# NVlabs/nvdiffrecmc

Measured on NVIDIA H100. Metric: shadow_rays_per_second_train_step, higher is better.
Workload: dtype f32

## Files before the change

### nvdiffrecmc_b200/csrc/envshade.cu

```cuda
#include "bsdf.cuh"
#include "bvh_traverse.cuh"
#include "ctx.h"
#include "exact.cuh"
#include <vector>

namespace {

constexpr float MIN_ROUGHNESS = 0.08f;

struct ShadeParams {
    TView pos, nrm, view, kd, ks, diff_grad, spec_grad;
    const float *light; int l_s1, l_s2, l_s3; int Hl, Wl;
    uint32_t *rec_count;
    float *rec_rays;
    int rec_slots;
    int B, H, W;
    uint32_t bsdf; float shadow_scale, sample_frac;
    float *pos_grad, *nrm_grad, *kd_grad, *ks_grad, *light_grad;
};

struct EnvParams : ShadeParams {
    TView mask, ro;
    const float *pdf; int p_s1, p_s2;
    const float *rows; int r_s;
// ... 103 lines not shown
__device__ __forceinline__ xf3 x_toworld(xf3 a, const PixelFrame &f) { return f.U * a.x + f.V * a.y + f.W * a.z; }

__device__ __forceinline__ float ggx_pdf_value(const PixelFrame &f, f3 wi)
{
    const f3 wo_l = toF3(f.wo_l_raw);
    const xf3 wi_lx = x_tolocal(X3(wi), f);
    const f3 wi_l = toF3(wi_lx);
    float pdf = 0.0f;
    if (wo_l.z > 0.0f && wi_l.z > 0.0f) {
        const f3 m = toF3(xnormalize(wi_lx + f.wo_l_raw));
        float woDotH = dot(m, wo_l);
        float alpha = f.alpha.v;
        float D = eval_ndf_ggx(alpha, m.z);
        float G1 = eval_g1_ggx(alpha * alpha, wo_l.z);
        pdf = G1 * D * fmaxf(0.0f, woDotH) / wo_l.z;
        pdf /= (4.0f * woDotH);
    }
    return pdf;
}
__device__ __forceinline__ void update_pdf(float &pdf, float opdf, float b) { if (b > 0.000001f) pdf += opdf * b; }

__device__ __forceinline__ float bsdf_pdf_value(const PixelFrame &f, xf3 wi)
{
    xf NdotL = xdot(f.N, wi);
    if (xmin(f.NdotV, NdotL).v < 1e-6f) return 1.0f;
    float pdf = 0.0f;
    float pD = f.pDiffuse.v;
    if (pD > 0.0f) update_pdf(pdf, fmaxf(NdotL.v, 0.0f) * MCS_INV_PI, pD);
    if (f.pSpecular.v > 0.0f) update_pdf(pdf, ggx_pdf_value(f, toF3(wi)), 1.0f - pD);
    return pdf;
}

__device__ __forceinline__ xf3 bsdf_sample(const PixelFrame &f, xf sx, xf sy, xf sz, float &pdf)
{
    pdf = 0.0f;
    const float pD = f.pDiffuse.v;
    xf3 wi;
    if (sz < f.pDiffuse) {
        if (pD < 0.0001f) { pdf = 1.0f; return f.N; }
        xf phi = xf(__double2float_rn(xd_mul(2.0 * XD_PI, (double)sx.v)));
        xf ct = xsqrt(sy);
        xf st = xf(__double2float_rn(__dsqrt_rn(__dsub_rn(1.0, (double)sy.v))));
        xf sp, cp;
        det_sincos(phi, sp, cp);
        xf3 vec = f.U * (cp * st) + f.V * (sp * st) + f.W * ct;
        wi = xnormalize(vec);
        pdf = fmaxf(0.000001f, ct.v * MCS_INV_PI) * pD;
        if (f.pSpecular.v > 0.0f) update_pdf(pdf, ggx_pdf_value(f, toF3(wi)), 1.0f - pD);
    } else {
        if (!(f.wo_l.z.v > 0.0f)) { pdf = 0.0f; wi = X3(xf(0.0f), xf(0.0f), xf(0.0f)); }
        else {
            const xf alpha = f.alpha;
            xf3 Vh = xnormalize(X3(alpha * f.wo_l.x, alpha * f.wo_l.y, f.wo_l.z));
            xf3 T1 = (Vh.z.v < 0.9999f) ? xnormalize(xcross(X3(xf(0.0f), xf(0.0f), xf(1.0f)), Vh)) : X3(xf(1.0f), xf(0.0f), xf(0.0f));
            xf3 T2 = xcross(Vh, T1);
            xf r = xsqrt(sx);
            xf phi = (xf(2.0f) * xf(MCS_PI)) * sy;
            xf sp, cp;
            det_sincos(phi, sp, cp);
            xf t1 = r * cp, t2 = r * sp;
            xf s = xf(0.5f) * (xf(1.0f) + Vh.z);
            t2 = (xf(1.0f) - s) * xsqrt(xf(1.0f) - t1 * t1) + s * t2;
            xf3 Nh = T1 * t1 + T2 * t2 + Vh * xsqrt(xmax(xf(0.0f), xf(1.0f) - t1 * t1 - t2 * t2));
            xf3 h = xnormalize(X3(alpha * Nh.x, alpha * Nh.y, xmax(xf(0.0f), Nh.z)));
            xf woDotH = xdot(f.wo_l, h);
            xf3 wi_l = h * woDotH * xf(2.0f) - f.wo_l;
            wi = xnormalize(x_toworld(wi_l, f));
            float a = alpha.v, woz = f.wo_l.z.v;
            float G1 = eval_g1_ggx(a * a, woz);
            float D = eval_ndf_ggx(a, h.z.v);
            pdf = G1 * D * fmaxf(0.0f, woDotH.v) / woz;
            pdf /= (4.0f * woDotH.v);
        }
        pdf *= 1.0f - pD;
        if (pD > 0.0f) update_pdf(pdf, fmaxf(xdot(f.N, wi).v, 0.0f) * MCS_INV_PI, pD);
    }
    return wi;
}

__device__ __forceinline__ float warp_sum(float v)
{
#pragma unroll
    for (int o = 16; o > 0; o >>= 1) v += __shfl_xor_sync(0xFFFFFFFFu, v, o);
    return v;
}

struct ShadeAcc { f3 D, S, kd, ks, nrm, wo; };

template <bool BWD>
__device__ __forceinline__ void shade_ray(const ShadeParams &p, const f3 nrm, const f3 kd, const f3 ks, const f3 wo, const f3 dgrad, const f3 sgrad,
                                          const f3 wi, const float mis, const uint32_t tex, ShadeAcc &a)
{
    const bool diffuse_only = (p.bsdf == 1u || p.bsdf == 2u);
    const int tx = tex & 0xFFFFu, ty = (tex >> 16) & 0x7FFFu;
    const float wgt = ((tex >> 31) ? 1.0f - p.shadow_scale : 1.0f) * mis * p.sample_frac;
    const float *lp = p.light + (size_t)ty * p.l_s1 + (size_t)tx * p.l_s2;
    const f3 light_col = F3(__ldg(lp), __ldg(lp + p.l_s3), __ldg(lp + 2 * p.l_s3));
    float diffv = 0.0f; f3 specv = F3(0.0f);
    if (!BWD) {
        if (diffuse_only) diffv = fwd_lambert(nrm, wi);
        else ox_fwd_pbr_bsdf(kd, ks, wo, nrm, wi, MIN_ROUGHNESS, diffv, specv);
        a.D += light_col * (diffv * wgt);
        a.S += specv * light_col * wgt;
        return;
    }
    const f3 dD = dgrad * light_col * wgt, dS = sgrad * light_col * wgt;
    ox_fwdbwd_pbr_bsdf(diffuse_only, kd, ks, wo, nrm, wi, MIN_ROUGHNESS, sum(dD), dS, diffv, specv, a.kd, a.ks, a.wo, a.nrm);
    const f3 lg = F3(__fmaf_rn(dgrad.x, diffv, __fmul_rn(sgrad.x, specv.x)), __fmaf_rn(dgrad.y, diffv, __fmul_rn(sgrad.y, specv.y)),
                     __fmaf_rn(dgrad.z, diffv, __fmul_rn(sgrad.z, specv.z))) * wgt;
    float *gp = p.light_grad + ((size_t)ty * p.Wl + tx) * 3;
    if (lg.x != 0.0f) atomicAdd(gp, lg.x);
    if (lg.y != 0.0f) atomicAdd(gp + 1, lg.y);
    if (lg.z != 0.0f) atomicAdd(gp + 2, lg.z);
}

__device__ __forceinline__ void store_pixel_grads(const ShadeParams &p, const int64_t pix, const f3 pos, const f3 view, const ShadeAcc &a, const int lane)
{
    const float v[12] = {a.kd.x, a.kd.y, a.kd.z, a.ks.x, a.ks.y, a.ks.z, a.nrm.x, a.nrm.y, a.nrm.z, a.wo.x, a.wo.y, a.wo.z};
    const bool b4 = (lane >> 4) & 1, b3 = (lane >> 3) & 1;
    float h[6], t[3];
#pragma unroll
    for (int i = 0; i < 6; ++i) h[i] = (b4 ? v[6 + i] : v[i]) + __shfl_xor_sync(0xFFFFFFFFu, b4 ? v[i] : v[6 + i], 16);
#pragma unroll
    for (int i = 0; i < 3; ++i) t[i] = (b3 ? h[3 + i] : h[i]) + __shfl_xor_sync(0xFFFFFFFFu, b3 ? h[i] : h[3 + i], 8);
#pragma unroll
    for (int o = 4; o > 0; o >>= 1) {
#pragma unroll
        for (int i = 0; i < 3; ++i) t[i] += __shfl_xor_sync(0xFFFFFFFFu, t[i], o);
    }
    if ((lane & 7) == 0) {
        const int which = lane >> 3;
        float *g = (which == 0 ? p.kd_grad : which == 1 ? p.ks_grad : which == 2 ? p.nrm_grad : p.pos_grad) + pix * 3;
        if (which == 3) {
            f3 d__wo = F3(0.0f);
            bwd_safe_normalize(view - pos, d__wo, F3(t[0], t[1], t[2]));
            t[0] = -d__wo.x; t[1] = -d__wo.y; t[2] = -d__wo.z;
        }
        g[0] = t[0]; g[1] = t[1]; g[2] = t[2];
    }
}

__device__ __forceinline__ void zero_pixel_grads(const ShadeParams &p, const int64_t pix)
{
    float *a = p.pos_grad + pix * 3, *b = p.nrm_grad + pix * 3, *c = p.kd_grad + pix * 3, *d = p.ks_grad + pix * 3;
    a[0] = a[1] = a[2] = 0.0f; b[0] = b[1] = b[2] = 0.0f; c[0] = c[1] = c[2] = 0.0f; d[0] = d[1] = d[2] = 0.0f;
}

#ifndef MCS_REPLAY_MINB
#define MCS_REPLAY_MINB 32
#endif
#ifndef MCS_CTA_WARPS
#define MCS_CTA_WARPS 8
#endif
#ifndef MCS_STREAM_RECORD
#define MCS_STREAM_RECORD 1
#endif
#ifndef MCS_SPLIT_WALKS
#define MCS_SPLIT_WALKS 1
#endif
#ifndef MCS_SPLIT_BELOW
#define MCS_SPLIT_BELOW 20
#endif
#ifndef MCS_QSTACK
#define MCS_QSTACK 100
#endif
#ifndef MCS_LEAF_BATCH
#define MCS_LEAF_BATCH 32
#endif
#ifndef MCS_REFILL_BELOW
#define MCS_REFILL_BELOW 24
#endif
#ifndef MCS_COUNT_TRAVERSAL
#define MCS_COUNT_TRAVERSAL 0
#endif
#if MCS_COUNT_TRAVERSAL
__device__ unsigned long long g_trace_counts[3];
#endif
constexpr int NW = MCS_CTA_WARPS;
constexpr int SEG = 128;
constexpr int QTOT = NW * SEG;
#ifndef MCS_PCAP
#define MCS_PCAP 160
#endif
constexpr int PCAP = MCS_PCAP;
constexpr int PIXRING = 256;
static_assert(QTOT <= 65536, "queue entry index is stored in 16 bits");
static_assert(SEG <= 256 && SEG % 32 == 0, "sample slot within a fill is stored in 8 bits");

struct BlockQueue {
    float dx[QTOT], dy[QTOT], dz[QTOT], mis[QTOT];
    uint32_t tex[QTOT];
    uint16_t vlist[QTOT];
    uint8_t qitem[QTOT];
    uint32_t hitw[NW][SEG / 32];
    uint2 pl[NW][PCAP];
    float ro[NW][3];
    float rog[NW][3];
    float wo[NW][3];
    int pixid[NW];
    int seg_cnt[NW];
    int seg_head[NW];
    int pixring[PIXRING];
    int ring_head, ring_tail, more_chunks;
};
struct BlockQueueRec { uint32_t slot[QTOT]; };

struct PixelIn {
    f3 ro, pos, nrm, view, kd, ks;
    int ix, iy, iz;
    int64_t pix;
};

__device__ __forceinline__ PixelIn load_pixel(const EnvParams &p, int64_t pix)
{
    PixelIn q;
    q.pix = pix;
    q.ix = (int)(pix % p.W);
    const int64_t tt = pix / p.W;
    q.iy = (int)(tt % p.H); q.iz = (int)(tt / p.H);
    q.ro = p.ro.ld3(q.iz, q.iy, q.ix);
    q.pos = p.pos.ld3(q.iz, q.iy, q.ix);
    q.nrm = p.nrm.ld3(q.iz, q.iy, q.ix);
    q.view = p.view.ld3(q.iz, q.iy, q.ix);
    q.kd = p.kd.ld3(q.iz, q.iy, q.ix);
    q.ks = p.ks.ld3(q.iz, q.iy, q.ix);
    return q;
}

__device__ __forceinline__ void make_frame(const PixelIn &q, PixelFrame &f)
{
    f.N = X3(q.nrm);
    f.alpha = xf(q.ks.y) * xf(q.ks.y);
    f.wo = xnormalize(X3(q.view) - X3(q.pos));
    xf metallic = xf(q.ks.z);
    xf3 base = X3(q.kd);
    xf om = xf(1.0f) - metallic;
    xf3 specColor = X3(xf(0.04f) * om + base.x * metallic, xf(0.04f) * om + base.y * metallic, xf(0.04f) * om + base.z * metallic);
    xf lum = base.x * xf(0.2126f) + base.y * xf(0.7152f) + base.z * xf(0.0722f);
    xf diffuseWeight = om * lum;
    f.W = xnormalize(f.N);
    xONB(f.W, f.U, f.V);
    f.wo_l_raw = x_tolocal(f.wo, f);
    f.wo_l = xnormalize(f.wo_l_raw);
    xf specularWeight = xf(0.0f);
    if (f.wo_l.z.v > 0.0f) {
        xf c = xclamp(f.wo_l.z, xf(1e-4f), xf(1.0f) - xf(1e-4f));
        xf o = xf(1.0f) - c;
        xf o2 = o * o;
        xf scale = (o2 * o2) * o;
        xf os = xf(1.0f) - scale;
        xf3 F = X3(specColor.x * os + scale, specColor.y * os + scale, specColor.z * os + scale);
        specularWeight = F.x * xf(0.2126f) + F.y * xf(0.7152f) + F.z * xf(0.0722f);
    }
    xf sumw = diffuseWeight + specularWeight;
    f.pDiffuse = sumw.v > 0.0f ? diffuseWeight / sumw : xf(1.0f);
    f.pSpecular = xf(1.0f) - f.pDiffuse;
    f.NdotV = xdot(f.N, f.wo);
}

struct RayQ {
    float ax, ay, az, bx, by, bz;
    uint32_t nx, ny, nz, fx, fy, fz;
};
__device__ __forceinline__ float rcp_approx(float x) { float r; asm("rcp.approx.ftz.f32 %0, %1;" : "=f"(r) : "f"(x)); return r; }
__device__ __forceinline__ RayQ rayq_fetch(const float *__restrict__ g, const float *rog, float dx, float dy, float dz)
{
    RayQ r;
    const float ix = rcp_approx(fabsf(dx) < 1e-20f ? copysignf(1e-20f, dx) : dx);
    const float iy = rcp_approx(fabsf(dy) < 1e-20f ? copysignf(1e-20f, dy) : dy);
    const float iz = rcp_approx(fabsf(dz) < 1e-20f ? copysignf(1e-20f, dz) : dz);
    r.ax = __ldg(g + 3) * ix; r.ay = __ldg(g + 4) * iy; r.az = __ldg(g + 5) * iz;
    r.bx = fmaf(-8388608.0f, r.ax, rog[0] * ix);
    r.by = fmaf(-8388608.0f, r.ay, rog[1] * iy);
    r.bz = fmaf(-8388608.0f, r.az, rog[2] * iz);
    r.nx = dx < 0.0f ? 0x7432u : 0x7410u; r.ny = dy < 0.0f ? 0x7432u : 0x7410u; r.nz = dz < 0.0f ? 0x7432u : 0x7410u;
    r.fx = dx < 0.0f ? 0x7410u : 0x7432u; r.fy = dy < 0.0f ? 0x7410u : 0x7432u; r.fz = dz < 0.0f ? 0x7410u : 0x7432u;
    return r;
}
__device__ __forceinline__ float qplane(uint32_t w, uint32_t sel)
{
    uint32_t r;
    asm("prmt.b32 %0, %1, %2, %3;" : "=r"(r) : "r"(w), "r"(0x4B000000u), "r"(sel));
    return __uint_as_float(r);
}
__device__ __forceinline__ bool qslab(const uint4 c, const RayQ &r)
{
    const float a0 = fmaf(qplane(c.x, r.nx), r.ax, r.bx), a1 = fmaf(qplane(c.x, r.fx), r.ax, r.bx);
    const float b0 = fmaf(qplane(c.y, r.ny), r.ay, r.by), b1 = fmaf(qplane(c.y, r.fy), r.ay, r.by);
    const float c0 = fmaf(qplane(c.z, r.nz), r.az, r.bz), c1 = fmaf(qplane(c.z, r.fz), r.az, r.bz);
    const float tn = fmaxf(fmaxf(a0, b0), fmaxf(c0, 0.0f));
    const float tf = fminf(fminf(a1, b1), c1);
    return tn <= tf;
}

template <int MODE>
__device__ __forceinline__ void gen_segment(const EnvParams &p, BlockQueue &q, BlockQueueRec *qr, const PixelIn &px, const PixelFrame &f,
                                            int seg, int w0, int w1, int &qn, const int lane)
{
    const int S = p.S;
    const int qb = seg * SEG;
    const xf strata_frac = xf(1.0f) / xf((float)(unsigned)p.N);
    uint32_t s_seed = p.seed + (p.seed_dev ? __ldg(p.seed_dev) : 0u), s_pix = (uint32_t)(((px.iz + p.batch_offset) * p.H + px.iy) * p.W + px.ix);
    uint32_t rng = rand_pcg(s_seed) ^ rand_pcg(s_pix);
    const uint32_t lightIdx = rand_pcg(rng) % p.n_perms;
    const uint32_t bsdfIdx = rand_pcg(rng) % p.n_perms;
    const uint32_t rng2 = rng;
    const f3 nrm = px.nrm;

    for (int base = w0; base < w1; base += 32) {
        const int w = base + lane;
        const bool valid = w < w1;
        const bool is_bsdf = w >= S;
        const int i = is_bsdf ? w - S : w;
        xf3 dir = X3(xf(0.0f), xf(0.0f), xf(1.0f));
        float pdf_sum = 1.0f, pdf_b = 0.0f;
        int tx = 0, ty = 0;
        if (valid) {
            const uint2 sk = __ldg(p.skip + 5 * i + (is_bsdf ? 2 : 0));
            uint32_t st = rng2 * sk.x + sk.y;
            const uint32_t row = is_bsdf ? bsdfIdx : lightIdx;
            const uint32_t perm = (uint32_t)__ldg(p.perms + (size_t)row * p.pm_s1 + (size_t)i * p.pm_s3);
            const xf sx = (xf((float)(perm % (uint32_t)p.N)) + uniform_pcg(st)) * strata_frac;
            const xf sy = (xf((float)(perm / (uint32_t)p.N)) + uniform_pcg(st)) * strata_frac;
            if (!is_bsdf) {
                uint32_t cyi, cxi;
                xf ry = sample_cdf(p.rows, p.r_s, p.Hl, p.m_rows, sy, cyi);
                xf rx = sample_cdf(p.cols + (size_t)cyi * p.c_s1, p.c_s2, p.Wl, p.m_cols, sx, cxi);
                dir = tc_to_dir((xf((float)cxi) + rx) / xf((float)p.Wl), (xf((float)cyi) + ry) / xf((float)p.Hl));
            } else {
                const xf sz = uniform_pcg(st);
                dir = bsdf_sample(f, sx, sy, sz, pdf_b);
            }
            if (MODE == 2) {
                float cy;
                dir_to_texel(p, dir, tx, ty, cy);
                pdf_sum = light_pdf_value(p, tx, ty, cy) + (is_bsdf ? pdf_b : bsdf_pdf_value(f, dir));
            }
        }
        const f3 wi = toF3(dir);
        const bool live = valid && dot(nrm, wi) > 0.0f;
        if (MODE == 2 && valid) {
            const size_t rec = (size_t)px.pix * (2 * S) + (size_t)(2 * i + (is_bsdf ? 1 : 0));
            p.rec_texel[rec] = (ty << 16) | tx;
            if (!live) p.rec_vis[rec] = 2;
        }
        const unsigned m = __ballot_sync(0xFFFFFFFFu, live);
        if (live) {
            const int e = qb + qn + __popc(m & ((1u << lane) - 1u));
            q.dx[e] = wi.x; q.dy[e] = wi.y; q.dz[e] = wi.z;
            if (MODE == 2) {
                q.mis[e] = 1.0f / fmaxf(pdf_sum, 0.0001f);
                q.tex[e] = (uint32_t)((ty << 16) | tx);
                qr->slot[e] = (uint32_t)(2 * i + (is_bsdf ? 1 : 0));
            } else {
                q.mis[e] = pdf_b;
                q.tex[e] = is_bsdf ? 1u : 0u;
            }
            q.qitem[e] = (uint8_t)(w - w0);
        }
        qn += __popc(m);
    }
    if (MODE != 2) {
        __syncwarp();
        for (int e0 = 0; e0 < qn; e0 += 32) {
            const int e = qb + e0 + lane;
            if (e0 + lane < qn) {
                const xf3 dir = X3(xf(q.dx[e]), xf(q.dy[e]), xf(q.dz[e]));
                int tx, ty; float cy;
                dir_to_texel(p, dir, tx, ty, cy);
                const float pdf_sum = light_pdf_value(p, tx, ty, cy) + (q.tex[e] ? q.mis[e] : bsdf_pdf_value(f, dir));
                q.mis[e] = 1.0f / fmaxf(pdf_sum, 0.0001f);
                q.tex[e] = (uint32_t)((ty << 16) | tx);
            }
        }
    }
}

__device__ __forceinline__ void trace_queue(const EnvParams &p, BlockQueue &q, const int warp, const int lane)
{
    constexpr int REFILL_BELOW = MCS_REFILL_BELOW;
    constexpr int LEAF_BATCH = MCS_LEAF_BATCH;
    unsigned lt;
    asm("mov.u32 %0, %%lanemask_lt;" : "=r"(lt));
    int pend = 0;
    int my = -1;
    int node = 0, sp = 0, sb = 0;
    int stack[MCS_QSTACK];
    RayQ r; r.ax = r.ay = r.az = 1.0f; r.bx = r.by = r.bz = 0.0f; r.nx = r.ny = r.nz = 0x7410u; r.fx = r.fy = r.fz = 0x7432u;
    const BvhView b = p.bvh;
    uint2 *pl = q.pl[warp];
    int seg = warp, exhausted = 0;
#if MCS_COUNT_TRAVERSAL
    unsigned long long n_rays = 0, n_visits = 0, n_tests = 0;
#endif

    auto leaf_batch = [&](int n) {
        __syncwarp();
        const int base = pend - n;
        if (lane < n) {
            const uint2 ent = pl[base + lane];
            const int e = (int)ent.x;
            if (!(q.tex[e] >> 31)) {
                const int code = (int)ent.y;
                const int start = code >> 3, cnt = (code & 7) + 1;
                const int ps = e / SEG;
                const f3 o = F3(q.ro[ps][0], q.ro[ps][1], q.ro[ps][2]);
                const f3 d = F3(q.dx[e], q.dy[e], q.dz[e]);
                bool hit = false;
                for (int k = 0; k < cnt && !hit; ++k) {
#if MCS_COUNT_TRAVERSAL
                    ++n_tests;
#endif
                    const float4 *t = b.tris + 3 * (size_t)(start + k);
                    const float4 t0 = __ldg(t), t1 = __ldg(t + 1), t2 = __ldg(t + 2);
                    float tt, uu, vv;
                    hit = mt_hit(o, d, F3(t0.x, t0.y, t0.z), F3(t1.x, t1.y, t1.z), F3(t2.x, t2.y, t2.z), MCS_TMAX, tt, uu, vv);
                }
                if (hit) atomicOr(&q.tex[e], 0x80000000u);
            }
        }
        pend = base;
        __syncwarp();
    };

    while (true) {
        unsigned idle = __ballot_sync(0xFFFFFFFFu, my < 0);
        while (idle && exhausted < NW) {
            const int need = __popc(idle);
            int base = 0;
            if (lane == 0) base = atomicAdd(&q.seg_head[seg], need);
            base = __shfl_sync(0xFFFFFFFFu, base, 0);
            const int avail = q.seg_cnt[seg] - base;
            if (avail <= 0) { seg = seg + 1 == NW ? 0 : seg + 1; ++exhausted; continue; }
            const int take = avail < need ? avail : need;
            const int rank = __popc(idle & lt);
            if (my < 0 && rank < take) {
                const int idx = seg * SEG + base + rank;
                my = idx;
                r = rayq_fetch(b.qgrid, q.rog[seg], q.dx[idx], q.dy[idx], q.dz[idx]);
                node = 0; sp = 0; sb = 0;
#if MCS_COUNT_TRAVERSAL
                ++n_rays;
#endif
            }
            if (take < need) { seg = seg + 1 == NW ? 0 : seg + 1; ++exhausted; }
            idle = __ballot_sync(0xFFFFFFFFu, my < 0);
        }
#if MCS_SPLIT_WALKS
        if (exhausted >= NW && idle) {
            const unsigned donors = __ballot_sync(0xFFFFFFFFu, my >= 0 && sp > sb);
            if (donors) {
                const int npair = min(__popc(idle), __popc(donors));
                uint2 *xch = pl + (PCAP - 32);
                const int kd = __popc(donors & lt), ki = __popc(idle & lt);
                if (my >= 0 && sp > sb && kd < npair) { xch[kd] = make_uint2((unsigned)my, (unsigned)stack[sb]); ++sb; }
                __syncwarp();
                if (my < 0 && ki < npair) {
                    const uint2 g = xch[ki];
                    my = (int)g.x; node = (int)g.y; sp = 0; sb = 0;
                    const int ps = my / SEG;
                    r = rayq_fetch(b.qgrid, q.rog[ps], q.dx[my], q.dy[my], q.dz[my]);
                }
                __syncwarp();
            }
        }
#endif
        int nact = __popc(__ballot_sync(0xFFFFFFFFu, my >= 0));
        if (nact == 0) {
            if (pend == 0) break;
            leaf_batch(pend < 32 ? pend : 32);
            continue;
        }
        const int thresh = exhausted < NW ? REFILL_BELOW : (MCS_SPLIT_WALKS ? MCS_SPLIT_BELOW : 1);
        do {
            const int cur = my;
            unsigned lmask = 0u;
            int c0 = 0, c1 = 0, c2 = 0, c3 = 0;
            if (my >= 0) {
#if MCS_COUNT_TRAVERSAL
                ++n_visits;
#endif
                const uint4 *n = b.nodesq4 + 4 * (size_t)node;
                const uint4 k0 = __ldg(n), k1 = __ldg(n + 1), k2 = __ldg(n + 2), k3 = __ldg(n + 3);
                const bool h0 = qslab(k0, r), h1 = qslab(k1, r), h2 = qslab(k2, r), h3 = qslab(k3, r);
                const unsigned hm = (h0 ? 1u : 0u) | (h1 ? 2u : 0u) | (h2 ? 4u : 0u) | (h3 ? 8u : 0u);
                const unsigned lb = k0.w >> 28;
                c0 = (int)(k0.w & 0x0FFFFFFFu); c1 = (int)k1.w; c2 = (int)k2.w; c3 = (int)k3.w;
                lmask = hm & lb;
                const unsigned im = hm & ~lb;
                stack[sp] = c0; sp += (int)(im & 1u);
                stack[sp] = c1; sp += (int)((im >> 1) & 1u);
                stack[sp] = c2; sp += (int)((im >> 2) & 1u);
                stack[sp] = c3; sp += (int)(im >> 3);
                if (im) { node = (im & 8u) ? c3 : ((im & 4u) ? c2 : ((im & 2u) ? c1 : c0)); --sp; }
                else if (sp > sb) node = stack[--sp];
                else my = -1;
            }
            for (unsigned mL = __ballot_sync(0xFFFFFFFFu, lmask != 0u); mL; mL = __ballot_sync(0xFFFFFFFFu, lmask != 0u)) {
                if (lmask) {
                    const unsigned low = lmask & (0u - lmask);
                    const int code = (low & 3u) ? ((low & 1u) ? c0 : c1) : ((low & 4u) ? c2 : c3);
                    pl[pend + __popc(mL & lt)] = make_uint2((unsigned)cur, (unsigned)code);
                    lmask ^= low;
                }
                pend += __popc(mL);
                if (PCAP < 160 && pend >= LEAF_BATCH) leaf_batch(32);
            }
            nact = __popc(__ballot_sync(0xFFFFFFFFu, my >= 0));
        } while (pend < LEAF_BATCH && nact >= thresh);
        while (pend >= LEAF_BATCH) leaf_batch(32);
        if (my >= 0 && (q.tex[my] >> 31)) my = -1;
    }
#if MCS_COUNT_TRAVERSAL
    atomicAdd(&g_trace_counts[0], n_rays); atomicAdd(&g_trace_counts[1], n_visits); atomicAdd(&g_trace_counts[2], n_tests);
#endif
    __syncwarp();
}

template <int MODE>
__global__ void __launch_bounds__(NW * 32, 32 / NW) env_shade_kernel(const EnvParams p)
{
    extern __shared__ __align__(16) unsigned char smem_raw[];
    const int lane = threadIdx.x & 31, warp = threadIdx.x >> 5;
    BlockQueue &q = *reinterpret_cast<BlockQueue *>(smem_raw);
    BlockQueueRec *qr = MODE == 2 ? reinterpret_cast<BlockQueueRec *>(smem_raw + sizeof(BlockQueue)) : nullptr;

    const int64_t npix = (int64_t)p.B * p.H * p.W;
    const unsigned int nchunks = (unsigned int)((npix + 31) / 32);
    const int S = p.S, items = 2 * S;
    const bool trace_needed = p.shadow_scale != 0.0f;
    const float v_occluded = 1.0f - p.shadow_scale;
    const int nsub = (items + SEG - 1) / SEG;
    const int qb = warp * SEG;

    if (threadIdx.x == 0) { q.ring_head = 0; q.ring_tail = 0; q.more_chunks = 1; }
    __syncthreads();

    while (true) {
        while (true) {
            const int have = q.ring_tail - q.ring_head;
            const int more = q.more_chunks;
            __syncthreads();
            if (have >= NW || !more) break;
            if (warp < (NW >= 16 ? 4 : 2)) {
                unsigned int chunk = 0;
                if (lane == 0) chunk = atomicAdd(p.chunk_counter, 1u);
                chunk = __shfl_sync(0xFFFFFFFFu, chunk, 0);
                if (chunk >= nchunks) { if (lane == 0) q.more_chunks = 0; }
                else {
                    const int64_t mypix = (int64_t)chunk * 32 + lane;
                    const bool mine = mypix < npix;
                    float mval = 0.0f;
                    if (mine) {
                        const int mx = (int)(mypix % p.W); const int64_t t = mypix / p.W;
                        mval = p.mask.ld1((int)(t / p.H), (int)(t % p.H), mx);
                    }
                    const bool act = mine && mval > 0.0f;
                    const unsigned am = __ballot_sync(0xFFFFFFFFu, act);
                    if (mine && !act) {
                        if (MODE != 1) {
                            float *d = p.diff + mypix * 3, *s = p.spec + mypix * 3;
                            d[0] = d[1] = d[2] = 0.0f; s[0] = s[1] = s[2] = 0.0f;
                            if (p.hit_out) for (int k = 0; k < p.hit_words; ++k) p.hit_out[(size_t)mypix * p.hit_words + k] = 0u;
                            if (p.rec_count) p.rec_count[mypix] = 0u;
                        } else zero_pixel_grads(p, mypix);
                    }
                    int base = 0;
                    if (lane == 0 && am) base = atomicAdd(&q.ring_tail, __popc(am));
                    base = __shfl_sync(0xFFFFFFFFu, base, 0);
                    if (act) q.pixring[(base + __popc(am & ((1u << lane) - 1u))) & (PIXRING - 1)] = (int)mypix;
                }
            }
            __syncthreads();
        }
        const int have = q.ring_tail - q.ring_head;
        if (have <= 0) break;
        const int nb = have < NW ? have : NW;
        const bool has_px = warp < nb;
        const int64_t mypx = has_px ? (int64_t)q.pixring[(q.ring_head + warp) & (PIXRING - 1)] : 0;
        __syncthreads();
        if (threadIdx.x == 0) q.ring_head += nb;

        ShadeAcc acc{};
        int rec_off = 0;

        for (int sub = 0; sub < nsub; ++sub) {
            const int w0 = sub * SEG, w1 = min(items, w0 + SEG);
            int qn = 0;
            if (has_px) {
                const PixelIn px = load_pixel(p, mypx);
                PixelFrame f;
                make_frame(px, f);
                if (lane < 3) {
                    const float ro_l = lane == 0 ? px.ro.x : (lane == 1 ? px.ro.y : px.ro.z);
                    q.rog[warp][lane] = __fsub_rn(__ldg(p.bvh.qgrid + lane), ro_l);
                    q.ro[warp][lane] = lane == 0 ? px.ro.x : (lane == 1 ? px.ro.y : px.ro.z);
                    q.wo[warp][lane] = lane == 0 ? f.wo.x.v : (lane == 1 ? f.wo.y.v : f.wo.z.v);
                }
                gen_segment<MODE>(p, q, qr, px, f, warp, w0, w1, qn, lane);
            }
            if (lane == 0) { q.seg_cnt[warp] = qn; q.seg_head[warp] = 0; q.pixid[warp] = (int)mypx; }
            __syncthreads();
            const bool replay = MODE == 1 && p.hit_in != nullptr;
            if (replay) {
                if (has_px) {
                    if (lane < SEG / 32) {
                        const int wi_ = w0 / 32 + lane;
                        q.hitw[warp][lane] = wi_ < p.hit_words ? __ldg(p.hit_in + (size_t)mypx * p.hit_words + wi_) : 0u;
                    }
                    __syncwarp();
                    for (int e = lane; e < qn; e += 32) {
                        const int it = q.qitem[qb + e];
                        if ((q.hitw[warp][it >> 5] >> (it & 31)) & 1u) q.tex[qb + e] |= 0x80000000u;
                    }
                }
            } else if (trace_needed) trace_queue(p, q, warp, lane);
            __syncthreads();
            if (MODE != 1 && p.hit_out != nullptr && has_px) {
                if (lane < SEG / 32) q.hitw[warp][lane] = 0u;
                __syncwarp();
                for (int e = lane; e < qn; e += 32)
                    if (q.tex[qb + e] >> 31) { const int it = q.qitem[qb + e]; atomicOr(&q.hitw[warp][it >> 5], 1u << (it & 31)); }
                __syncwarp();
                if (lane < SEG / 32) {
                    const int wi_ = w0 / 32 + lane;
                    if (wi_ < p.hit_words) p.hit_out[(size_t)mypx * p.hit_words + wi_] = q.hitw[warp][lane];
                }
            }
            if (has_px) {
                if (MODE == 2) {
                    for (int e = lane; e < qn; e += 32) {
                        const size_t rec = (size_t)mypx * items + qr->slot[qb + e];
                        p.rec_vis[rec] = trace_needed ? (uint8_t)(1u - (q.tex[qb + e] >> 31)) : (uint8_t)2;
                    }
                }
                int vn = 0;
                for (int e0 = 0; e0 < qn; e0 += 32) {
                    const int e = e0 + lane;
                    const bool keep = e < qn && (!(q.tex[qb + e] >> 31) || v_occluded != 0.0f);
                    const unsigned m = __ballot_sync(0xFFFFFFFFu, keep);
                    if (keep) q.vlist[qb + vn + __popc(m & ((1u << lane) - 1u))] = (uint16_t)(qb + e);
                    vn += __popc(m);
                }
                __syncwarp();
                if (MODE != 1 && p.rec_count != nullptr) {
                    float *rr = p.rec_rays + (size_t)mypx * 5 * p.rec_slots;
                    for (int k = lane; k < vn; k += 32) {
                        const int e = q.vlist[qb + k];
                        const int o = rec_off + k;
#if MCS_STREAM_RECORD
                        __stcs(rr + o, q.dx[e]); __stcs(rr + p.rec_slots + o, q.dy[e]); __stcs(rr + 2 * p.rec_slots + o, q.dz[e]);
                        __stcs(rr + 3 * p.rec_slots + o, q.mis[e]); __stcs(rr + 4 * p.rec_slots + o, __uint_as_float(q.tex[e]));
#else
                        rr[o] = q.dx[e]; rr[p.rec_slots + o] = q.dy[e]; rr[2 * p.rec_slots + o] = q.dz[e]; rr[3 * p.rec_slots + o] = q.mis[e];
                        rr[4 * p.rec_slots + o] = __uint_as_float(q.tex[e]);
#endif
                    }
                    rec_off += vn;
                    if (sub == nsub - 1 && lane == 0) p.rec_count[mypx] = (uint32_t)rec_off;
                }
                const PixelIn px = load_pixel(p, mypx);
                const f3 wo_f = F3(q.wo[warp][0], q.wo[warp][1], q.wo[warp][2]);
                f3 dgrad = F3(0.0f), sgrad = F3(0.0f);
                if (MODE == 1) { dgrad = p.diff_grad.ld3(px.iz, px.iy, px.ix); sgrad = p.spec_grad.ld3(px.iz, px.iy, px.ix); }

                for (int k = lane; k < vn; k += 32) {
                    const int e = q.vlist[qb + k];
                    shade_ray<MODE == 1>(p, px.nrm, px.kd, px.ks, wo_f, dgrad, sgrad, F3(q.dx[e], q.dy[e], q.dz[e]), q.mis[e], q.tex[e], acc);
                }

                if (sub == nsub - 1) {
                    if (MODE != 1) {
                        float r0 = warp_sum(acc.D.x), r1 = warp_sum(acc.D.y), r2 = warp_sum(acc.D.z);
                        float r3 = warp_sum(acc.S.x), r4 = warp_sum(acc.S.y), r5 = warp_sum(acc.S.z);
                        if (lane == 0) {
                            float *d = p.diff + px.pix * 3, *s = p.spec + px.pix * 3;
                            d[0] = r0; d[1] = r1; d[2] = r2; s[0] = r3; s[1] = r4; s[2] = r5;
                        }
                    } else store_pixel_grads(p, px.pix, px.pos, px.view, acc, lane);
                }
            }
            __syncthreads();
        }
    }
}

__global__ void __launch_bounds__(32, MCS_REPLAY_MINB) env_shade_replay_kernel(const ShadeParams p)
{
    const int lane = threadIdx.x;
    const int64_t npix = (int64_t)p.B * p.H * p.W;
    for (int64_t chunk = blockIdx.x; chunk * 32 < npix; chunk += gridDim.x) {
        const int64_t mypix = chunk * 32 + lane;
        const uint32_t mycnt = mypix < npix ? __ldg(p.rec_count + mypix) : 0u;
        unsigned rem = __ballot_sync(0xFFFFFFFFu, mycnt != 0u);
        if (mypix < npix && mycnt == 0u) zero_pixel_grads(p, mypix);
        while (rem) {
            const int src = __ffs(rem) - 1;
            rem &= rem - 1;
            const int64_t pix = chunk * 32 + src;
            const int cnt = (int)__shfl_sync(0xFFFFFFFFu, mycnt, src);
            const int ix = (int)(pix % p.W); const int64_t tt = pix / p.W; const int iy = (int)(tt % p.H), iz = (int)(tt / p.H);
            const f3 pos = p.pos.ld3(iz, iy, ix), nrm = p.nrm.ld3(iz, iy, ix), view = p.view.ld3(iz, iy, ix), kd = p.kd.ld3(iz, iy, ix), ks = p.ks.ld3(iz, iy, ix);
            const f3 dgrad = p.diff_grad.ld3(iz, iy, ix), sgrad = p.spec_grad.ld3(iz, iy, ix);
            const f3 wo_f = safe_normalize(view - pos);
            const float *rr = p.rec_rays + (size_t)pix * 5 * p.rec_slots;
            ShadeAcc acc{};
            for (int k = lane; k < cnt; k += 32) {
#if MCS_STREAM_RECORD
                const f3 wi = F3(__ldcs(rr + k), __ldcs(rr + p.rec_slots + k), __ldcs(rr + 2 * p.rec_slots + k));
                const float mis = __ldcs(rr + 3 * p.rec_slots + k);
                const uint32_t tex = __float_as_uint(__ldcs(rr + 4 * p.rec_slots + k));
#else
                const f3 wi = F3(__ldg(rr + k), __ldg(rr + p.rec_slots + k), __ldg(rr + 2 * p.rec_slots + k));
                const float mis = __ldg(rr + 3 * p.rec_slots + k);
                const uint32_t tex = __float_as_uint(__ldg(rr + 4 * p.rec_slots + k));
#endif
                shade_ray<true>(p, nrm, kd, ks, wo_f, dgrad, sgrad, wi, mis, tex, acc);
            }
            store_pixel_grads(p, pix, pos, view, acc, lane);
        }
    }
}

__global__ void k_skip_table(uint2 *__restrict__ tab, int n)
{
    const int k = blockIdx.x * blockDim.x + threadIdx.x;
    if (k >= n) return;
    uint32_t m = 1u, a = 0u;
    uint32_t bm = 747796405u, ba = 2891336453u;
    for (uint32_t e = (uint32_t)k; e; e >>= 1) {
        if (e & 1u) { a = a * bm + ba; m = m * bm; }
        ba = ba * bm + ba; bm = bm * bm;
    }
    tab[k] = make_uint2(m, a);
}

static int ensure_skip_table(mcs_ctx *c, int N, cudaStream_t s, const uint2 **out)
{
    for (int i = 0; i < c->n_skip; ++i)
        if (c->skip_N[i] == N) { *out = (const uint2 *)c->lcg_skip[i].p; return 0; }
    const int slot = c->n_skip < MCS_SKIP_TABLES ? c->n_skip : (c->skip_evict++ % MCS_SKIP_TABLES);
    const int n = 5 * N * N + 3;
    if (int e = mcs_buf_reserve(c->lcg_skip[slot], sizeof(uint2) * (size_t)n + 16, s)) return e;
    k_skip_table<<<(n + 255) / 256, 256, 0, s>>>((uint2 *)c->lcg_skip[slot].p, n);
    MCS_LAUNCH_CHECK();
    c->skip_N[slot] = N;
    if (c->n_skip < MCS_SKIP_TABLES) ++c->n_skip;
    *out = (const uint2 *)c->lcg_skip[slot].p;
    return 0;
}

static int cdf_iters(int size)
{
    int steps = 0;
    for (int span = size - 1; span > 0; span = span / 4) ++steps;
    return steps + 1;
}

static void fill_shade_params(ShadeParams &p, const mcs_tensor *extent, const mcs_tensor *gb_pos, const mcs_tensor *gb_normal,
                              const mcs_tensor *gb_view_pos, const mcs_tensor *gb_kd, const mcs_tensor *gb_ks, const mcs_tensor *light,
                              uint32_t bsdf, uint32_t n_samples_x, float shadow_scale)
{
    p.B = extent->sizes[0]; p.H = extent->sizes[1]; p.W = extent->sizes[2];
    p.pos = make_view(gb_pos); p.nrm = make_view(gb_normal); p.view = make_view(gb_view_pos); p.kd = make_view(gb_kd); p.ks = make_view(gb_ks);
    p.Hl = light->sizes[1]; p.Wl = light->sizes[2];
    p.light = (const float *)light->ptr; p.l_s1 = light->strides[1]; p.l_s2 = light->strides[2]; p.l_s3 = light->strides[3];
    p.bsdf = bsdf; p.shadow_scale = shadow_scale;
    p.sample_frac = 1.0f / (float)(n_samples_x * n_samples_x);
}

static int set_grad_outputs(ShadeParams &p, const mcs_tensor *diff_grad, const mcs_tensor *spec_grad, float *gb_pos_grad, float *gb_normal_grad,
                            float *gb_kd_grad, float *gb_ks_grad, float *light_grad, cudaStream_t s)
{
    p.diff_grad = make_view(diff_grad); p.spec_grad = make_view(spec_grad);
    p.pos_grad = gb_pos_grad; p.nrm_grad = gb_normal_grad; p.kd_grad = gb_kd_grad; p.ks_grad = gb_ks_grad; p.light_grad = light_grad;
    MCS_CUDA(cudaMemsetAsync(light_grad, 0, sizeof(float) * 3 * (size_t)p.Hl * p.Wl, s));
    return 0;
}

static int fill_params(mcs_ctx *ctx, EnvParams &p,
                       const mcs_tensor *mask, const mcs_tensor *ro, const mcs_tensor *gb_pos, const mcs_tensor *gb_normal,
                       const mcs_tensor *gb_view_pos, const mcs_tensor *gb_kd, const mcs_tensor *gb_ks,
                       const mcs_tensor *light, const mcs_tensor *pdf, const mcs_tensor *rows, const mcs_tensor *cols,
                       const mcs_tensor *perms, uint32_t bsdf, uint32_t n_samples_x, uint32_t rnd_seed, const uint32_t *seed_offset_dev, float shadow_scale, int32_t batch_offset,
                       cudaStream_t s)
{
    MCS_REQUIRE(ctx != nullptr, "env_shade: null context");
    MCS_REQUIRE(ctx->T > 0, "env_shade: no acceleration structure built (call optix_build_bvh first)");
    const mcs_tensor *all[] = {mask, ro, gb_pos, gb_normal, gb_view_pos, gb_kd, gb_ks, light, pdf, rows, cols, perms};
    for (const mcs_tensor *t : all) MCS_REQUIRE(view_ok(t), "env_shade: null / empty tensor argument");
    MCS_REQUIRE(bsdf <= 2u, "env_shade: BSDF must be 0 ('pbr'), 1 ('diffuse') or 2 ('white')");
    MCS_REQUIRE(n_samples_x >= 1u && n_samples_x <= 64u, "env_shade: n_samples_x must be in [1, 64]");
    fill_shade_params(p, ro, gb_pos, gb_normal, gb_view_pos, gb_kd, gb_ks, light, bsdf, n_samples_x, shadow_scale);
    MCS_REQUIRE(ro->sizes[3] == 3, "env_shade: ro must be [B,H,W,3]");
    MCS_REQUIRE((int64_t)p.B * p.H * p.W < (1ll << 31) / 3, "env_shade: launch too large for 32-bit indexing");
    const mcs_tensor *gb[] = {mask, gb_pos, gb_normal, gb_view_pos, gb_kd, gb_ks};
    const char *gbn[] = {"mask", "gb_pos", "gb_normal", "gb_view_pos", "gb_kd", "gb_ks"};
    for (int i = 0; i < 6; ++i) {
        for (int d = 0; d < 3; ++d)
            MCS_REQUIRE(gb[i]->sizes[d] == ro->sizes[d] || gb[i]->sizes[d] == 1, "env_shade: %s dim %d = %d is not broadcastable to %d", gbn[i], d,
                        gb[i]->sizes[d], ro->sizes[d]);
        MCS_REQUIRE(gb[i]->sizes[3] == (i == 0 ? 1 : 3) || gb[i]->sizes[3] == 1, "env_shade: %s has a bad channel count %d", gbn[i], gb[i]->sizes[3]);
    }
    p.mask = make_view(mask); p.ro = make_view(ro);
    MCS_REQUIRE(light->sizes[3] == 3 && p.Hl >= 2 && p.Wl >= 2, "env_shade: light must be [Hl>=2, Wl>=2, 3]");
    MCS_REQUIRE(p.Hl < 32768 && p.Wl < 65536, "env_shade: light probe too large");
    MCS_REQUIRE(pdf->sizes[1] == p.Hl && pdf->sizes[2] == p.Wl && cols->sizes[1] == p.Hl && cols->sizes[2] == p.Wl && rows->sizes[1] == p.Hl,
                "env_shade: pdf / rows / cols do not match the light probe resolution");
    p.pdf = (const float *)pdf->ptr; p.p_s1 = pdf->strides[1]; p.p_s2 = pdf->strides[2];
    p.rows = (const float *)rows->ptr; p.r_s = rows->strides[1];
    p.cols = (const float *)cols->ptr; p.c_s1 = cols->strides[1]; p.c_s2 = cols->strides[2];
    p.N = (int)n_samples_x; p.S = p.N * p.N;
    p.hit_words = (2 * p.S + 31) / 32;
    MCS_REQUIRE(perms->sizes[3] == p.S && perms->sizes[1] >= 1, "env_shade: perms must be [P, n_samples_x^2]");
    p.perms = (const int32_t *)perms->ptr; p.pm_s1 = perms->strides[1]; p.pm_s3 = perms->strides[3]; p.n_perms = (uint32_t)perms->sizes[1];
    p.m_rows = cdf_iters(p.Hl); p.m_cols = cdf_iters(p.Wl);
    p.seed = rnd_seed; p.seed_dev = seed_offset_dev; p.batch_offset = batch_offset;
    p.bvh = ctx->shadow;
    p.bvh.nodes = (const float4 *)ctx->nodes.p;
    if (int e = ensure_skip_table(ctx, p.N, s, &p.skip)) return e;
    if (int e = mcs_buf_reserve(ctx->counters, MCS_COUNTER_RING * 64, s)) return e;
    p.chunk_counter = (unsigned int *)((char *)ctx->counters.p + 64 * (size_t)(ctx->counter_next++ % MCS_COUNTER_RING));
    MCS_CUDA(cudaMemsetAsync(p.chunk_counter, 0, sizeof(unsigned int), s));
    return 0;
}

template <int MODE>
static int launch_env(const EnvParams &p, cudaStream_t s)
{
    int dev = 0, sms = 0, per_sm = 0;
    MCS_CUDA(cudaGetDevice(&dev));
    MCS_CUDA(cudaDeviceGetAttribute(&sms, cudaDevAttrMultiProcessorCount, dev));
    const size_t smem = sizeof(BlockQueue) + (MODE == 2 ? sizeof(BlockQueueRec) : 0);
    MCS_CUDA(cudaFuncSetAttribute(env_shade_kernel<MODE>, cudaFuncAttributeMaxDynamicSharedMemorySize, (int)smem));
    {
        const size_t need = (size_t)(32 / NW) * (smem + 1024);
        int pct = (int)((need * 100 + 228 * 1024 - 1) / (228 * 1024));
        MCS_CUDA(cudaFuncSetAttribute(env_shade_kernel<MODE>, cudaFuncAttributePreferredSharedMemoryCarveout, pct > 100 ? 100 : pct));
    }
    MCS_CUDA(cudaOccupancyMaxActiveBlocksPerMultiprocessor(&per_sm, env_shade_kernel<MODE>, NW * 32, smem));
    if (per_sm < 1) per_sm = 1;
    const int64_t npix = (int64_t)p.B * p.H * p.W;
    int64_t want = (npix + 32 * NW - 1) / (32 * NW);
    int grid = (int)(want < (int64_t)sms * per_sm ? want : (int64_t)sms * per_sm);
    if (grid < 1) grid = 1;
    env_shade_kernel<MODE><<<grid, NW * 32, smem, s>>>(p);
    MCS_LAUNCH_CHECK();
    return 0;
}

}

extern "C" {

int mcs_env_shade_fwd(mcs_ctx *ctx,
                      const mcs_tensor *mask, const mcs_tensor *ro, const mcs_tensor *gb_pos, const mcs_tensor *gb_normal,
                      const mcs_tensor *gb_view_pos, const mcs_tensor *gb_kd, const mcs_tensor *gb_ks,
                      const mcs_tensor *light, const mcs_tensor *pdf, const mcs_tensor *rows, const mcs_tensor *cols,
                      const mcs_tensor *perms,
                      uint32_t bsdf, uint32_t n_samples_x, uint32_t rnd_seed, const uint32_t *seed_offset_dev, float shadow_scale, int32_t batch_offset,
                      float *diff, float *spec, uint32_t *hit_record, uint32_t *rec_count, float *rec_rays, int32_t rec_slots, mcs_stream stream)
{
    EnvParams p{};
    cudaStream_t s = (cudaStream_t)stream;
    if (int e = fill_params(ctx, p, mask, ro, gb_pos, gb_normal, gb_view_pos, gb_kd, gb_ks, light, pdf, rows, cols, perms, bsdf, n_samples_x, rnd_seed,
                            seed_offset_dev, shadow_scale, batch_offset, s)) return e;
    MCS_REQUIRE(diff && spec, "env_shade_fwd: null output pointer");
    p.diff = diff; p.spec = spec; p.hit_out = hit_record;
    MCS_REQUIRE((rec_count == nullptr) == (rec_rays == nullptr), "env_shade_fwd: rec_count and rec_rays go together");
    MCS_REQUIRE(rec_count == nullptr || rec_slots >= 2 * p.S, "env_shade_fwd: rec_slots must be >= 2 * n_samples_x^2");
    p.rec_count = rec_count; p.rec_rays = rec_rays; p.rec_slots = rec_slots;
    return launch_env<0>(p, s);
}

int mcs_env_shade_records(mcs_ctx *ctx,
                          const mcs_tensor *mask, const mcs_tensor *ro, const mcs_tensor *gb_pos, const mcs_tensor *gb_normal,
                          const mcs_tensor *gb_view_pos, const mcs_tensor *gb_kd, const mcs_tensor *gb_ks,
                          const mcs_tensor *light, const mcs_tensor *pdf, const mcs_tensor *rows, const mcs_tensor *cols,
                          const mcs_tensor *perms,
                          uint32_t bsdf, uint32_t n_samples_x, uint32_t rnd_seed, const uint32_t *seed_offset_dev, float shadow_scale, int32_t batch_offset,
                          float *diff, float *spec, int32_t *rec_texel, uint8_t *rec_vis, mcs_stream stream)
{
    EnvParams p{};
    cudaStream_t s = (cudaStream_t)stream;
    if (int e = fill_params(ctx, p, mask, ro, gb_pos, gb_normal, gb_view_pos, gb_kd, gb_ks, light, pdf, rows, cols, perms, bsdf, n_samples_x, rnd_seed,
                            seed_offset_dev, shadow_scale, batch_offset, s)) return e;
    MCS_REQUIRE(diff && spec && rec_texel && rec_vis, "env_shade_records: null output pointer");
    p.diff = diff; p.spec = spec; p.rec_texel = rec_texel; p.rec_vis = rec_vis;
    return launch_env<2>(p, s);
}

int mcs_env_shade_bwd(mcs_ctx *ctx,
                      const mcs_tensor *mask, const mcs_tensor *ro, const mcs_tensor *gb_pos, const mcs_tensor *gb_normal,
                      const mcs_tensor *gb_view_pos, const mcs_tensor *gb_kd, const mcs_tensor *gb_ks,
                      const mcs_tensor *light, const mcs_tensor *pdf, const mcs_tensor *rows, const mcs_tensor *cols,
                      const mcs_tensor *perms,
                      uint32_t bsdf, uint32_t n_samples_x, uint32_t rnd_seed, const uint32_t *seed_offset_dev, float shadow_scale, int32_t batch_offset,
                      const mcs_tensor *diff_grad, const mcs_tensor *spec_grad,
                      float *gb_pos_grad, float *gb_normal_grad, float *gb_kd_grad, float *gb_ks_grad, float *light_grad,
                      const uint32_t *hit_record, mcs_stream stream)
{
    EnvParams p{};
    cudaStream_t s = (cudaStream_t)stream;
    if (int e = fill_params(ctx, p, mask, ro, gb_pos, gb_normal, gb_view_pos, gb_kd, gb_ks, light, pdf, rows, cols, perms, bsdf, n_samples_x, rnd_seed,
                            seed_offset_dev, shadow_scale, batch_offset, s)) return e;
    MCS_REQUIRE(view_ok(diff_grad) && view_ok(spec_grad), "env_shade_bwd: null / empty upstream gradient");
    MCS_REQUIRE(gb_pos_grad && gb_normal_grad && gb_kd_grad && gb_ks_grad && light_grad, "env_shade_bwd: null output pointer");
    for (int d = 0; d < 3; ++d)
        MCS_REQUIRE(diff_grad->sizes[d] == ro->sizes[d] && spec_grad->sizes[d] == ro->sizes[d], "env_shade_bwd: upstream gradient shape mismatch");
    if (int e = set_grad_outputs(p, diff_grad, spec_grad, gb_pos_grad, gb_normal_grad, gb_kd_grad, gb_ks_grad, light_grad, s)) return e;
    p.hit_in = hit_record;
    return launch_env<1>(p, s);
}

int mcs_env_shade_bwd_replay(const mcs_tensor *gb_pos, const mcs_tensor *gb_normal, const mcs_tensor *gb_view_pos, const mcs_tensor *gb_kd,
                             const mcs_tensor *gb_ks, const mcs_tensor *light, uint32_t bsdf, uint32_t n_samples_x, float shadow_scale,
                             const mcs_tensor *diff_grad, const mcs_tensor *spec_grad, const uint32_t *rec_count, const float *rec_rays, int32_t rec_slots,
                             float *gb_pos_grad, float *gb_normal_grad, float *gb_kd_grad, float *gb_ks_grad, float *light_grad, mcs_stream stream)
{
    cudaStream_t s = (cudaStream_t)stream;
    const mcs_tensor *all[] = {gb_pos, gb_normal, gb_view_pos, gb_kd, gb_ks, light, diff_grad, spec_grad};
    for (const mcs_tensor *t : all) MCS_REQUIRE(view_ok(t), "env_shade_bwd_replay: null / empty tensor argument");
    MCS_REQUIRE(rec_count && rec_rays && rec_slots > 0, "env_shade_bwd_replay: missing ray record");
    MCS_REQUIRE(gb_pos_grad && gb_normal_grad && gb_kd_grad && gb_ks_grad && light_grad, "env_shade_bwd_replay: null output pointer");
    MCS_REQUIRE(bsdf <= 2u && n_samples_x >= 1u, "env_shade_bwd_replay: bad bsdf / n_samples_x");
    ShadeParams p{};
    fill_shade_params(p, diff_grad, gb_pos, gb_normal, gb_view_pos, gb_kd, gb_ks, light, bsdf, n_samples_x, shadow_scale);
    p.rec_count = const_cast<uint32_t *>(rec_count); p.rec_rays = const_cast<float *>(rec_rays); p.rec_slots = rec_slots;
    if (int e = set_grad_outputs(p, diff_grad, spec_grad, gb_pos_grad, gb_normal_grad, gb_kd_grad, gb_ks_grad, light_grad, s)) return e;
    const int64_t npix = (int64_t)p.B * p.H * p.W;
    const int64_t chunks = (npix + 31) / 32;
    const int grid = (int)(chunks < INT32_MAX ? chunks : INT32_MAX);
    env_shade_replay_kernel<<<grid, 32, 0, s>>>(p);
    MCS_LAUNCH_CHECK();
    return 0;
}

#if MCS_COUNT_TRAVERSAL
int mcs_trace_counts(unsigned long long *out, int reset)
{
    MCS_CUDA(cudaDeviceSynchronize());
    MCS_CUDA(cudaMemcpyFromSymbol(out, g_trace_counts, sizeof(g_trace_counts)));
    if (reset) {
        const unsigned long long zero[3] = {0, 0, 0};
        MCS_CUDA(cudaMemcpyToSymbol(g_trace_counts, zero, sizeof(zero)));
    }
    return 0;
}
#endif

}
```

Before: 6741.

## Shrink shared queue, drop far-plane selectors, tune forward CTAs per SM and carveout

Puts the per-warp pixel list into a union with the visibility list and hit words, halves the pixel ring for small CTAs and removes the unused pixid array, all to shrink shared memory per block. Computes the far-plane byte selectors by XOR from the near ones, cutting three registers per ray. Sets the forward kernel's launch bound to 4 CTAs per SM and rounds the shared-memory carveout up to the hardware step sizes. Also adds optional per-phase clock instrumentation that is compiled out by default. The union is only safe if the pixel list and the vlist/hitw data are never live at the same time.

Measured after the change: 6793, median of 6. No clear change (+0.8%).

```diff
diff --git a/nvdiffrecmc_b200/csrc/envshade.cu b/nvdiffrecmc_b200/csrc/envshade.cu
--- a/nvdiffrecmc_b200/csrc/envshade.cu
+++ b/nvdiffrecmc_b200/csrc/envshade.cu
@@ -279,6 +279,9 @@
 #ifndef MCS_CTA_WARPS
 #define MCS_CTA_WARPS 8
 #endif
+#ifndef MCS_FWD_CTAS
+#define MCS_FWD_CTAS 4
+#endif
 #ifndef MCS_STREAM_RECORD
 #define MCS_STREAM_RECORD 1
 #endif
@@ -303,32 +306,58 @@
 #if MCS_COUNT_TRAVERSAL
 __device__ unsigned long long g_trace_counts[3];
 #endif
+#ifndef MCS_PHASE_CLOCKS
+#define MCS_PHASE_CLOCKS 0
+#endif
+enum { PC_COLLECT, PC_SYNC_COLLECT, PC_SYNC_PICK, PC_GEN_A, PC_GEN_B, PC_SYNC_G, PC_TRACE, PC_SYNC_T, PC_EVAL, PC_SYNC_E, PC_N };
+#if MCS_PHASE_CLOCKS
+__device__ unsigned long long g_phase_clocks[PC_N];
+#endif
 constexpr int NW = MCS_CTA_WARPS;
+__host__ __device__ constexpr int ctas_per_sm(int mode) { return mode == 0 ? MCS_FWD_CTAS : 32 / NW; }
 constexpr int SEG = 128;
 constexpr int QTOT = NW * SEG;
 #ifndef MCS_PCAP
 #define MCS_PCAP 160
 #endif
 constexpr int PCAP = MCS_PCAP;
-constexpr int PIXRING = 256;
+constexpr int PIXRING = NW >= 16 ? 256 : 128;
+static_assert(PIXRING >= NW - 1 + 32 * (NW >= 16 ? 4 : 2), "pixel ring too small");
 static_assert(QTOT <= 65536, "queue entry index is stored in 16 bits");
 static_assert(SEG <= 256 && SEG % 32 == 0, "sample slot within a fill is stored in 8 bits");
 
 struct BlockQueue {
     float dx[QTOT], dy[QTOT], dz[QTOT], mis[QTOT];
     uint32_t tex[QTOT];
-    uint16_t vlist[QTOT];
     uint8_t qitem[QTOT];
-    uint32_t hitw[NW][SEG / 32];
-    uint2 pl[NW][PCAP];
+    union {
+        uint2 pl[NW][PCAP];
+        struct {
+            uint16_t vlist[QTOT];
+            uint32_t hitw[NW][SEG / 32];
+        };
+    };
     float ro[NW][3];
     float rog[NW][3];
     float wo[NW][3];
-    int pixid[NW];
     int seg_cnt[NW];
     int seg_head[NW];
     int pixring[PIXRING];
     int ring_head, ring_tail, more_chunks;
+#if MCS_PHASE_CLOCKS
+    unsigned long long pclk[NW][PC_N];
+#endif
+};
+
+struct PhaseClock {
+#if MCS_PHASE_CLOCKS
+    unsigned long long *acc; unsigned t0; bool lead;
+    __device__ __forceinline__ PhaseClock(BlockQueue &q, int warp, int lane) : acc(q.pclk[warp]), t0((unsigned)clock()), lead(lane == 0) {}
+    __device__ __forceinline__ void mark(int k) { const unsigned t = (unsigned)clock(); if (lead) acc[k] += t - t0; t0 = t; }
+#else
+    __device__ __forceinline__ PhaseClock(BlockQueue &, int, int) {}
+    __device__ __forceinline__ void mark(int) {}
+#endif
 };
 struct BlockQueueRec { uint32_t slot[QTOT]; };
 
@@ -387,7 +416,7 @@
 
 struct RayQ {
     float ax, ay, az, bx, by, bz;
-    uint32_t nx, ny, nz, fx, fy, fz;
+    uint32_t nx, ny, nz;
 };
 __device__ __forceinline__ float rcp_approx(float x) { float r; asm("rcp.approx.ftz.f32 %0, %1;" : "=f"(r) : "f"(x)); return r; }
 __device__ __forceinline__ RayQ rayq_fetch(const float *__restrict__ g, const float *rog, float dx, float dy, float dz)
@@ -401,7 +430,6 @@
     r.by = fmaf(-8388608.0f, r.ay, rog[1] * iy);
     r.bz = fmaf(-8388608.0f, r.az, rog[2] * iz);
     r.nx = dx < 0.0f ? 0x7432u : 0x7410u; r.ny = dy < 0.0f ? 0x7432u : 0x7410u; r.nz = dz < 0.0f ? 0x7432u : 0x7410u;
-    r.fx = dx < 0.0f ? 0x7410u : 0x7432u; r.fy = dy < 0.0f ? 0x7410u : 0x7432u; r.fz = dz < 0.0f ? 0x7410u : 0x7432u;
     return r;
 }
 __device__ __forceinline__ float qplane(uint32_t w, uint32_t sel)
@@ -412,9 +440,9 @@
 }
 __device__ __forceinline__ bool qslab(const uint4 c, const RayQ &r)
 {
-    const float a0 = fmaf(qplane(c.x, r.nx), r.ax, r.bx), a1 = fmaf(qplane(c.x, r.fx), r.ax, r.bx);
-    const float b0 = fmaf(qplane(c.y, r.ny), r.ay, r.by), b1 = fmaf(qplane(c.y, r.fy), r.ay, r.by);
-    const float c0 = fmaf(qplane(c.z, r.nz), r.az, r.bz), c1 = fmaf(qplane(c.z, r.fz), r.az, r.bz);
+    const float a0 = fmaf(qplane(c.x, r.nx), r.ax, r.bx), a1 = fmaf(qplane(c.x, r.nx ^ 0x22u), r.ax, r.bx);
+    const float b0 = fmaf(qplane(c.y, r.ny), r.ay, r.by), b1 = fmaf(qplane(c.y, r.ny ^ 0x22u), r.ay, r.by);
+    const float c0 = fmaf(qplane(c.z, r.nz), r.az, r.bz), c1 = fmaf(qplane(c.z, r.nz ^ 0x22u), r.az, r.bz);
     const float tn = fmaxf(fmaxf(a0, b0), fmaxf(c0, 0.0f));
     const float tf = fminf(fminf(a1, b1), c1);
     return tn <= tf;
@@ -422,7 +450,7 @@
 
 template <int MODE>
 __device__ __forceinline__ void gen_segment(const EnvParams &p, BlockQueue &q, BlockQueueRec *qr, const PixelIn &px, const PixelFrame &f,
-                                            int seg, int w0, int w1, int &qn, const int lane)
+                                            int seg, int w0, int w1, int &qn, const int lane, PhaseClock &pc)
 {
     const int S = p.S;
     const int qb = seg * SEG;
@@ -487,6 +515,7 @@
         }
         qn += __popc(m);
     }
+    pc.mark(PC_GEN_A);
     if (MODE != 2) {
         __syncwarp();
         for (int e0 = 0; e0 < qn; e0 += 32) {
@@ -513,7 +542,7 @@
     int my = -1;
     int node = 0, sp = 0, sb = 0;
     int stack[MCS_QSTACK];
-    RayQ r; r.ax = r.ay = r.az = 1.0f; r.bx = r.by = r.bz = 0.0f; r.nx = r.ny = r.nz = 0x7410u; r.fx = r.fy = r.fz = 0x7432u;
+    RayQ r; r.ax = r.ay = r.az = 1.0f; r.bx = r.by = r.bz = 0.0f; r.nx = r.ny = r.nz = 0x7410u;
     const BvhView b = p.bvh;
     uint2 *pl = q.pl[warp];
     int seg = warp, exhausted = 0;
@@ -645,7 +674,7 @@
 }
 
 template <int MODE>
-__global__ void __launch_bounds__(NW * 32, 32 / NW) env_shade_kernel(const EnvParams p)
+__global__ void __launch_bounds__(NW * 32, ctas_per_sm(MODE)) env_shade_kernel(const EnvParams p)
 {
     extern __shared__ __align__(16) unsigned char smem_raw[];
     const int lane = threadIdx.x & 31, warp = threadIdx.x >> 5;
@@ -661,13 +690,19 @@
     const int qb = warp * SEG;
 
     if (threadIdx.x == 0) { q.ring_head = 0; q.ring_tail = 0; q.more_chunks = 1; }
+#if MCS_PHASE_CLOCKS
+    for (int i = threadIdx.x; i < NW * PC_N; i += blockDim.x) q.pclk[i / PC_N][i % PC_N] = 0ull;
+#endif
     __syncthreads();
+    PhaseClock pc(q, warp, lane);
 
     while (true) {
         while (true) {
             const int have = q.ring_tail - q.ring_head;
             const int more = q.more_chunks;
+            pc.mark(PC_COLLECT);
             __syncthreads();
+            pc.mark(PC_SYNC_COLLECT);
             if (have >= NW || !more) break;
             if (warp < (NW >= 16 ? 4 : 2)) {
                 unsigned int chunk = 0;
@@ -698,14 +733,18 @@
                     if (act) q.pixring[(base + __popc(am & ((1u << lane) - 1u))) & (PIXRING - 1)] = (int)mypix;
                 }
             }
+            pc.mark(PC_COLLECT);
             __syncthreads();
+            pc.mark(PC_SYNC_COLLECT);
         }
         const int have = q.ring_tail - q.ring_head;
         if (have <= 0) break;
         const int nb = have < NW ? have : NW;
         const bool has_px = warp < nb;
         const int64_t mypx = has_px ? (int64_t)q.pixring[(q.ring_head + warp) & (PIXRING - 1)] : 0;
+        pc.mark(PC_COLLECT);
         __syncthreads();
+        pc.mark(PC_SYNC_PICK);
         if (threadIdx.x == 0) q.ring_head += nb;
 
         ShadeAcc acc{};
@@ -724,10 +763,12 @@
                     q.ro[warp][lane] = lane == 0 ? px.ro.x : (lane == 1 ? px.ro.y : px.ro.z);
                     q.wo[warp][lane] = lane == 0 ? f.wo.x.v : (lane == 1 ? f.wo.y.v : f.wo.z.v);
                 }
-                gen_segment<MODE>(p, q, qr, px, f, warp, w0, w1, qn, lane);
-            }
-            if (lane == 0) { q.seg_cnt[warp] = qn; q.seg_head[warp] = 0; q.pixid[warp] = (int)mypx; }
+                gen_segment<MODE>(p, q, qr, px, f, warp, w0, w1, qn, lane, pc);
+            }
+            if (lane == 0) { q.seg_cnt[warp] = qn; q.seg_head[warp] = 0; }
+            pc.mark(PC_GEN_B);
             __syncthreads();
+            pc.mark(PC_SYNC_G);
             const bool replay = MODE == 1 && p.hit_in != nullptr;
             if (replay) {
                 if (has_px) {
@@ -742,7 +783,9 @@
                     }
                 }
             } else if (trace_needed) trace_queue(p, q, warp, lane);
+            pc.mark(PC_TRACE);
             __syncthreads();
+            pc.mark(PC_SYNC_T);
             if (MODE != 1 && p.hit_out != nullptr && has_px) {
                 if (lane < SEG / 32) q.hitw[warp][lane] = 0u;
                 __syncwarp();
@@ -807,9 +850,19 @@
                     } else store_pixel_grads(p, px.pix, px.pos, px.view, acc, lane);
                 }
             }
+            pc.mark(PC_EVAL);
             __syncthreads();
-        }
-    }
+            pc.mark(PC_SYNC_E);
+        }
+    }
+#if MCS_PHASE_CLOCKS
+    __syncthreads();
+    if (threadIdx.x < PC_N) {
+        unsigned long long t = 0;
+        for (int w = 0; w < NW; ++w) t += q.pclk[w][threadIdx.x];
+        atomicAdd(&g_phase_clocks[threadIdx.x], t);
+    }
+#endif
 }
 
 __global__ void __launch_bounds__(32, MCS_REPLAY_MINB) env_shade_replay_kernel(const ShadeParams p)
@@ -961,9 +1014,12 @@
     const size_t smem = sizeof(BlockQueue) + (MODE == 2 ? sizeof(BlockQueueRec) : 0);
     MCS_CUDA(cudaFuncSetAttribute(env_shade_kernel<MODE>, cudaFuncAttributeMaxDynamicSharedMemorySize, (int)smem));
     {
-        const size_t need = (size_t)(32 / NW) * (smem + 1024);
-        int pct = (int)((need * 100 + 228 * 1024 - 1) / (228 * 1024));
-        MCS_CUDA(cudaFuncSetAttribute(env_shade_kernel<MODE>, cudaFuncAttributePreferredSharedMemoryCarveout, pct > 100 ? 100 : pct));
+        const size_t need = (size_t)ctas_per_sm(MODE) * (smem + 1024);
+        static const int step_kb[] = {0, 8, 16, 32, 64, 100, 132, 164, 196, 228};
+        int kb = 228;
+        for (int k : step_kb)
+            if ((size_t)k * 1024 >= need) { kb = k; break; }
+        MCS_CUDA(cudaFuncSetAttribute(env_shade_kernel<MODE>, cudaFuncAttributePreferredSharedMemoryCarveout, kb * 100 / 228));
     }
     MCS_CUDA(cudaOccupancyMaxActiveBlocksPerMultiprocessor(&per_sm, env_shade_kernel<MODE>, NW * 32, smem));
     if (per_sm < 1) per_sm = 1;
@@ -1063,6 +1119,19 @@
     return 0;
 }
 
+#if MCS_PHASE_CLOCKS
+int mcs_phase_clocks(unsigned long long *out, int reset)
+{
+    MCS_CUDA(cudaDeviceSynchronize());
+    MCS_CUDA(cudaMemcpyFromSymbol(out, g_phase_clocks, sizeof(g_phase_clocks)));
+    if (reset) {
+        const unsigned long long zero[PC_N] = {};
+        MCS_CUDA(cudaMemcpyToSymbol(g_phase_clocks, zero, sizeof(zero)));
+    }
+    return 0;
+}
+#endif
+
 #if MCS_COUNT_TRAVERSAL
 int mcs_trace_counts(unsigned long long *out, int reset)
 {
```
